# countertype/brotli-lib

Measured on AMD Instinct MI355X. Metric: encode+decode MB/s at q11 lgwin=22, higher is better.
Workload: dtype u8; 1 GPU; C4 per-GPU shard: 1024 x 1048576 B enwik-style text, q11 lgwin22 GENERIC, encode -> decode round trip (statuses and sizes checked); streams_per_gpu=1024, quality=11, lgwin=22, mode=0, parallelism=shard1

## Files before the change

brotli-lib_amd/csrc/enc_common.h:

```cpp
#pragma once
#include <hip/hip_runtime.h>
#include <stdint.h>

#include "common.h"
#include "parts.h"

#ifndef RFC_CONST
#define RFC_CONST static __device__ const
#endif
#include "rfc_tables.h"

namespace mib {
namespace enc {

constexpr uint32_t kSegBits = 16;
constexpr uint32_t kSeg = 1u << kSegBits;
#ifndef MIB_MAX_MATCHES
#define MIB_MAX_MATCHES 4
#endif
constexpr int kMaxMatches = MIB_MAX_MATCHES;
static_assert(kMaxMatches == 4 || kMaxMatches == 6 || kMaxMatches == 8, "records of 4, 6 or 8 entries");
constexpr int kMatchRec = kMaxMatches;
constexpr uint32_t kMatchLenSat = 255;
constexpr int kLongCopy = 200;
// ... 336 lines not shown
}
__device__ __forceinline__ uint32_t switch_bits(const Codes &cd, int cat, const Unit &u) {
  const int bc = block_count_code(u.sw_count[cat]);
  return cd.btd[cat][u.sw_code[cat]] + cd.bcd[cat][bc] + kBlkBits[bc];
}
__device__ __forceinline__ bool switch_at(const Unit &u, int cat, uint32_t q) { return u.sw_count[cat] && q == u.first[cat]; }
__device__ __forceinline__ bool lit_switch_at(const Unit &u, uint32_t lp) { return u.sw_count[0] && lp == u.first[0]; }

__device__ __forceinline__ uint32_t item_count(const Cmd &c) { return c.ins + 2; }

__device__ __forceinline__ uint32_t header_bits(const Codes &cd, const Cmd &c, const Unit &u, uint32_t q) {
  const int ic = ins_code(c.ins);
  const int cc = copy_code(c.copy ? c.copy : 2);
  uint32_t bits = cd.cd[u.type[1]][c.cmd_prefix] + kInsExtra[ic] + kCopyExtra[cc];
  if (switch_at(u, 1, q)) bits += switch_bits(cd, 1, u);
  return bits;
}
__device__ __forceinline__ int literal_tree(const uint16_t *cmap, const uint8_t *lut, const Unit &u, uint32_t p12) {
  return cmap[u.type[0] * kLitCtx + (lut[p12 & 0xFF] | lut[256 + (p12 >> 8)])];
}
__device__ __forceinline__ uint32_t dist_bits(const Codes &cd, const Mb &mb, const Cmd &c, const Unit &u, uint32_t q) {
  if (!c.copy || c.cmd_prefix < 128) return 0;
  uint32_t bits = cd.dd[mb.dist_cmap[u.type[2] * kDistCtx + dist_ctx(c.copy)]][c.dist_prefix & 0x3FF] + (c.dist_prefix >> 10);
  if (switch_at(u, 2, q)) bits += switch_bits(cd, 2, u);
  return bits;
}
__device__ __forceinline__ uint32_t item_bits(const Codes &cd, const Mb &mb, const uint16_t *cmap, const uint8_t *lut, const Job &jb,
                                              const Cmd &c, uint32_t p, const Seg &sg, const Unit *su, uint32_t q,
                                              uint32_t k) {
  if (k == 0) return header_bits(cd, c, su[unit_of(sg, p)], q);
  if (k > c.ins) return dist_bits(cd, mb, c, su[unit_of(sg, p)], q);
  const uint32_t lp = p + k - 1;
  const Unit &ul = su[unit_of(sg, lp)];
  return (lit_switch_at(ul, lp) ? switch_bits(cd, 0, ul) : 0u) + cd.ld[literal_tree(cmap, lut, ul, prev2(jb, lp))][jb.data[lp]];
}

template <int B>
struct ItemMap {
  uint32_t off[B + 1];
  __device__ __forceinline__ uint32_t find(uint32_t i, uint32_t nb) const {
    uint32_t lo = 0, hi = nb;
    while (hi - lo > 1) {
      const uint32_t mid = (lo + hi) >> 1;
      if (off[mid] <= i) lo = mid;
      else hi = mid;
    }
    return lo;
  }
};

void launch_dict_matches(hipStream_t st, const Job *jobs, int njobs, uint32_t span, const uint32_t *dict_tab,
                         const uint8_t *dict_data, uint32_t *matches);
void launch_cdict_matches(hipStream_t st, const Job *jobs, const uint32_t *pos_job, uint32_t total, uint32_t *matches);
void launch_find_matches(hipStream_t st, const Job *jobs, const uint32_t *pos_job, const SegRef *seg_ref,
                         const uint32_t *skeys, const uint32_t *svals, uint32_t total, int depth, uint32_t max_dist,
                         bool hist, bool parts, uint32_t *matches);
void launch_near_matches(hipStream_t st, const Job *jobs, const uint32_t *pos_job, const SegRef *seg_ref, uint32_t total,
                         uint32_t max_dist, bool hist, bool parts, uint32_t *matches);
void launch_lit_histo(hipStream_t st, const Job *jobs, const Seg *segs, int nsegs, uint32_t *lit_h);
void launch_hist_update(hipStream_t st, const Job *jobs, const uint32_t *pos_job, const uint32_t *skeys,
                        const uint32_t *svals, uint32_t total);
size_t cost_model_hist_bytes(int njobs);
void launch_cost_model(hipStream_t st, const Job *jobs, int njobs, const Seg *segs, int nsegs, const RawCmd *raw,
                       uint32_t *hist, CostModel *model);
void launch_dp(hipStream_t st, const Job *jobs, const Seg *segs, int nsegs, const uint32_t *lit_h, const CostModel *model,
               const uint32_t *matches, uint64_t *choice, bool cdict, bool font, const uint32_t *words, uint32_t *ring_hist,
               const Mb *mbs, int piece_shift);
void dp_launch_counts(unsigned long long out[4]);
size_t dp_ring_hist_bytes(int nsegs);
void launch_any_binary(hipStream_t st, const Job *jobs, int njobs, uint32_t *flag);
void launch_words(hipStream_t st, const Job *jobs, const uint32_t *pos_job, const SegRef *seg_ref, uint32_t total, uint32_t *words);
void launch_backtrack(hipStream_t st, const Job *jobs, Seg *segs, int nsegs, const uint64_t *choice, RawCmd *raw);
void launch_carry(hipStream_t st, Job *jobs, int njobs, Seg *segs, const Mb *mbs);
void launch_derive_segs(hipStream_t st, const Seg *segs, int nsegs, uint32_t sample, Seg *d_sample, Seg *pieces);
void launch_merge_pieces(hipStream_t st, const Job *jobs, Seg *segs, int nsegs, const Seg *pieces, RawCmd *raw);
void launch_rep(hipStream_t st, const Job *jobs, Seg *segs, int nsegs, const CostModel *model, RawCmd *raw, uint32_t *cnts);
size_t sort_ws_bytes(uint32_t total);
void launch_sort(hipStream_t st, const Job *jobs, const uint32_t *pos_job, int njobs, uint32_t total, int hb, void *ws,
                 uint32_t *tmp_k, uint32_t *tmp_v, uint32_t *skeys, uint32_t *svals);
void launch_codes(hipStream_t st, const Job *jobs, const Seg *segs, const Mb *mbs, int nsegs, const RawCmd *raw, Cmd *cmds,
                  uint32_t *cmd_pos, Unit *units, uint32_t *unit_h);
void launch_split(hipStream_t st, hipStream_t side, const Job *jobs, Mb *mbs, int nmbs, Unit *units,
                  const uint32_t *unit_h, Codes *codes, int max_units, int max_short_units);
void launch_histo(hipStream_t st, const Job *jobs, const Seg *segs, const Mb *mbs, int nsegs, const Cmd *cmds,
                  const uint32_t *cmd_pos, const Unit *units, uint32_t *hl, uint32_t *hc, uint32_t *hd);
void launch_dist_ring(hipStream_t st, Job *jobs, int njobs, const Seg *segs, const Cmd *cmds);
void launch_context_mode(hipStream_t st, const Job *jobs, Mb *mbs, int nmbs);
void launch_cluster(hipStream_t st, const Job *jobs, Mb *mbs, int nmbs, uint32_t *hl, uint32_t *hd);
void launch_huffman(hipStream_t st, hipStream_t side, const Job *jobs, Mb *mbs, int nmbs, const uint32_t *hl,
                    const uint32_t *hc, const uint32_t *hd, Codes *codes, uint8_t *trees, uint8_t *hdr);
void launch_sizes(hipStream_t st, const Job *jobs, Seg *segs, const Mb *mbs, int nsegs, const Cmd *cmds,
                  const uint32_t *cmd_pos, const Codes *codes, const Unit *units, uint32_t *tile_bits);
void launch_offsets(hipStream_t st, Job *jobs, int njobs, Mb *mbs, Seg *segs, uint8_t *out);
void launch_emit(hipStream_t st, const Job *jobs, const Mb *mbs, int nmbs, const Seg *segs, int nsegs, const Cmd *cmds,
                 const uint32_t *cmd_pos, const Codes *codes, const Unit *units, const uint32_t *tile_bits,
                 const uint8_t *trees, const uint8_t *hdr, uint8_t *out);
void launch_stored(hipStream_t st, Job *jobs, int njobs, uint8_t *out);
struct PushSum;
void launch_ring_scan(hipStream_t st, Job *jobs, int njobs, Seg *segs, int nsegs, const RawCmd *raw, PushSum *push);
void launch_part_index(hipStream_t st, const Job *jobs, int njobs, const Mb *mbs, const Seg *segs, int nsegs,
                       const Cmd *cmds, const Unit *units, PushSum *push, uint8_t *out);
size_t part_push_bytes();
void launch_pack(hipStream_t st, const Job *jobs, int njobs, uint64_t out_pos, uint64_t out_cap, uint64_t *dst_off,
                 const uint8_t *src, uint8_t *dst);

}
}
```

brotli-lib_amd/csrc/enc_entropy.hip:

```cpp
#include <hipcub/hipcub.hpp>
#include <cstdlib>
#include <algorithm>

#include "enc_common.h"

namespace mib {
namespace enc {

__global__ __launch_bounds__(64) void carry_kernel(Job *jobs, int njobs, Seg *segs, const Mb *mbs) {
  const int j = blockIdx.x, lane = threadIdx.x;
  if (j >= njobs) return;
  Job &jb = jobs[j];
  if (jb.uncompressed) return;
  uint32_t pd = (uint32_t)jb.dc_in[0];
  for (uint32_t m = 0; m < jb.nmb; m++) {
    const Mb &mb = mbs[jb.mb_base + m];
    uint32_t carry = 0;
    const uint32_t end = mb.first_seg + mb.nseg;
    for (uint32_t c0 = mb.first_seg; c0 < end; c0 += 64) {
      const uint32_t s = c0 + lane;
      const bool live = s < end;
      uint32_t ncmd = 0, tail = 0, last = 0;
      if (live) {
        ncmd = segs[s].ncmd;
// ... 138 lines not shown
    const uint32_t off = (uint32_t)(ex >> 35), total = (uint32_t)(tot >> 35);
    const uint32_t loff = (uint32_t)(ex >> 10) & 0x1FFFFFFu, nlits = (uint32_t)(tot >> 10) & 0x1FFFFFFu;
    const uint32_t rank = (uint32_t)ex & 0x3FFu, npush = (uint32_t)tot & 0x3FFu;
    const uint32_t pos = sh_run + off;
    if (push) sh_push[rank] = d;
    __syncthreads();
    uint32_t ring[4];
#pragma unroll
    for (int k = 0; k < 4; k++) ring[k] = (int)rank - 1 - k >= 0 ? sh_push[rank - 1 - k] : sh_ring[k - rank];
    uint32_t ring_after = 0;
    if (t < 4) ring_after = (int)npush - 1 - t >= 0 ? sh_push[npush - 1 - t] : sh_ring[t - npush];
    __syncthreads();
    if (t < 4) sh_ring[t] = ring_after;
    if (t == 0) sh_run += total;
    if (q < n) {
      Cmd c;
      c.ins = ins;
      c.copy = len;
      c.dist = d;
      c.dist_extra = 0;
      c.dist_prefix = 0;
      const int ic = ins_code(ins);
      const uint32_t u = unit_of(sg, pos);
      uint32_t *hu = sh_h + u * kSubHist;
      if (len) {
        const uint32_t dcode = is_word(jb, d) ? (d & ~kDictFlag) + 15 : d == prevd ? 0 : short_code(d, ring);
        uint32_t extra;
        const uint32_t dp = dist_prefix(dcode, (int)jb.ndirect, (int)jb.npostfix, &extra);
        c.dist_extra = extra;
        c.dist_prefix = (uint16_t)dp;
        c.cmd_prefix = (uint16_t)combine_codes(ic, copy_code(len), dcode == 0);
        if (c.cmd_prefix >= 128) {
          atomicAdd(&hu[256 + 704 + (dp & 0x3FF)], 1u);
          atomicAdd(&sh_n[u][2], 1u);
          atomicMin(&sh_first[u][2], q);
        }
      } else {
        c.cmd_prefix = (uint16_t)combine_codes(ic, 0, ic < 8);
      }
      atomicAdd(&hu[256 + c.cmd_prefix], 1u);
      atomicAdd(&sh_n[u][1], 1u);
      atomicMin(&sh_first[u][1], q);
      if (ins) {
        const uint32_t ulo = unit_of(sg, pos), uhi = unit_of(sg, pos + ins - 1);
        for (uint32_t v = ulo; v <= uhi; v++) {
          const uint32_t s0 = v == ulo ? pos : sg.start + (v << kSubBits);
          const uint32_t s1 = v == uhi ? pos + ins : sg.start + ((v + 1) << kSubBits);
          atomicAdd(&sh_n[v][0], s1 - s0);
          atomicMin(&sh_first[v][0], s0);
        }
      }
      out[q] = c;
      outp[q] = pos;
    }
    sh_pos[t] = pos;
    const uint32_t nb = min((uint32_t)NT, n - base);
    map.off[t] = loff;
    if (t == 0) map.off[nb] = nlits;
    __syncthreads();
    for (uint32_t i = t; i < nlits; i += NT) {
      const uint32_t j = map.find(i, nb);
      const uint32_t lp = sh_pos[j] + i - map.off[j];
      atomicAdd(&sh_h[unit_of(sg, lp) * kSubHist + jb.data[lp]], 1u);
    }
    __syncthreads();
  }
  const uint32_t u0 = blockIdx.x * kSubPerSeg;
  uint32_t *gh = unit_h + (size_t)u0 * kSubHist;
  for (int i = t; i < kSubPerSeg * kSubHist; i += NT) gh[i] = sh_h[i];
  if (t < kSubPerSeg) {
    Unit un;
    for (int c = 0; c < 3; c++) {
      un.nsym[c] = sh_n[t][c];
      un.first[c] = sh_first[t][c];
      un.sw_count[c] = 0;
      un.type[c] = 0;
      un.sw_code[c] = 0;
    }
    un.pad = 0;
    units[u0 + t] = un;
  }
}

template <int NT>
__global__ __launch_bounds__(NT) void histo_kernel(const Job *jobs, const Seg *segs, const Mb *mbs, const Cmd *cmds,
                                                       const uint32_t *cmd_pos, const Unit *units, uint32_t *hl,
                                                       uint32_t *hc, uint32_t *hd) {
  typedef hipcub::BlockScan<uint32_t, NT> Scan;
  __shared__ typename Scan::TempStorage scan_tmp;
  __shared__ uint32_t sh_l[kLitCtx * 256];
  __shared__ uint8_t ut[kSubPerSeg][3];
  __shared__ ItemMap<NT> map;
  __shared__ uint32_t sh_pos[NT], sh_ins[NT];
  uint32_t *sh_c = sh_l, *sh_d = sh_l + kMaxBT * 704;
  const Seg &sg = segs[blockIdx.x];
  const Job &jb = jobs[sg.job];
  if (jb.uncompressed) return;
  const Mb &mb = mbs[sg.mb];
  const int t = threadIdx.x;
  __shared__ uint8_t lut[512];
  for (int i = t; i < 512; i += NT) lut[i] = kRfcContextLut[(mb.ctx_mode << 9) + i];
  const Unit *un = units + (size_t)blockIdx.x * kSubPerSeg;
  if (t < kSubPerSeg * 3) ut[t / 3][t % 3] = un[t / 3].type[t % 3];
  for (int i = t; i < (int)mb.nbt[1] * 704; i += NT) sh_c[i] = 0;
  for (int i = t; i < (int)mb.nbt[2] * kDistCtx * 128; i += NT) sh_d[i] = 0;
  __syncthreads();
  const Cmd *c = cmds + sg.cmd_off;
  const uint32_t *cp = cmd_pos + sg.cmd_off;
  const uint32_t n = sg.ncmd + (sg.extra_ins ? 1 : 0);
  for (uint32_t q = t; q < n; q += NT) {
    const Cmd k = c[q];
    const uint32_t u = unit_of(sg, cp[q]);
    atomicAdd(&sh_c[ut[u][1] * 704 + k.cmd_prefix], 1u);
    if (k.copy && k.cmd_prefix >= 128) atomicAdd(&sh_d[(ut[u][2] * kDistCtx + dist_ctx(k.copy)) * 128 + (k.dist_prefix & 0x3FF)], 1u);
  }
  const uint32_t m = sg.mb;
  __syncthreads();
  for (int i = t; i < (int)mb.nbt[1] * 704; i += NT)
    if (sh_c[i]) atomicAdd(&hc[(size_t)m * kMaxBT * 704 + i], sh_c[i]);
  for (int i = t; i < (int)mb.nbt[2] * kDistCtx * 128; i += NT)
    if (sh_d[i]) atomicAdd(&hd[(size_t)m * kMaxBT * kDistCtx * 128 + i], sh_d[i]);
  __syncthreads();
  uint32_t present = 0;
  for (int u = 0; u < kSubPerSeg; u++) present |= 1u << ut[u][0];
  for (int ty = 0; ty < kMaxBT; ty++) {
    if (!(present >> ty & 1)) continue;
    for (int i = t; i < kLitCtx * 256; i += NT) sh_l[i] = 0;
    __syncthreads();
    for (uint32_t base = 0; base < n; base += NT) {
      const uint32_t q = base + t, nb = min((uint32_t)NT, n - base);
      uint32_t cnt = 0;
      if (q < n && c[q].ins) {
        const uint32_t pos = cp[q], ins = c[q].ins;
        sh_pos[t] = pos;
        sh_ins[t] = ins;
        const uint32_t ulo = unit_of(sg, pos), uhi = unit_of(sg, pos + ins - 1);
        for (uint32_t v = ulo; v <= uhi; v++)
          if (ut[v][0] == ty) {
            const uint32_t s0 = v == ulo ? pos : sg.start + (v << kSubBits);
            const uint32_t s1 = v == uhi ? pos + ins : sg.start + ((v + 1) << kSubBits);
            cnt += s1 - s0;
          }
      }
      uint32_t off, nlits;
      Scan(scan_tmp).ExclusiveSum(cnt, off, nlits);
      map.off[t] = off;
      if (t == 0) map.off[nb] = nlits;
      __syncthreads();
      for (uint32_t i = t; i < nlits; i += NT) {
        const uint32_t j = map.find(i, nb);
        const uint32_t pos = sh_pos[j], ins = sh_ins[j];
        const uint32_t ulo = unit_of(sg, pos), uhi = unit_of(sg, pos + ins - 1);
        uint32_t k = i - map.off[j], lp = pos;
        for (uint32_t v = ulo; v <= uhi; v++) {
          if (ut[v][0] != ty) continue;
          const uint32_t s0 = v == ulo ? pos : sg.start + (v << kSubBits);
          const uint32_t s1 = v == uhi ? pos + ins : sg.start + ((v + 1) << kSubBits);
          if (k < s1 - s0) {
            lp = s0 + k;
            break;
          }
          k -= s1 - s0;
        }
        const uint32_t p12 = prev2(jb, lp);
        atomicAdd(&sh_l[(lut[p12 & 0xFF] | lut[256 + (p12 >> 8)]) * 256 + jb.data[lp]], 1u);
      }
      __syncthreads();
    }
    uint32_t *dst = hl + ((size_t)m * kLitSlots + ty * kLitCtx) * 256;
    for (int i = t; i < kLitCtx * 256; i += NT)
      if (sh_l[i]) atomicAdd(&dst[i], sh_l[i]);
    __syncthreads();
  }
}

__device__ __forceinline__ float hist_cost(float bits, int nnz) {
  if (nnz <= 1) return 12.f;
  if (nnz <= 4) return bits + 20.f + 4.f * nnz;
  return bits + 40.f + 3.5f * nnz;
}

constexpr int kCluT = 1024;
constexpr int kCluPairs = kLitCtx * (kLitCtx - 1) / 2;
__device__ __forceinline__ int tri(int a, int b) { return a * (2 * kLitCtx - a - 1) / 2 + b - a - 1; }
#ifdef MIB_PROF
__device__ unsigned long long g_clu_prof[8];
#endif
__global__ __launch_bounds__(kCluT) void cluster_kernel(const Job *jobs, Mb *mbs, int nmbs, uint32_t *hl, uint32_t *hd,
                                                         int lit_cap, int kl, int kd) {
  constexpr int kMaxH = kLitCtx;
  __shared__ uint32_t h[kMaxH][257];
  __shared__ float cost[kMaxH];
  __shared__ float save[kCluPairs];
  __shared__ uint16_t pair_of[kCluPairs];
  __shared__ int alive[kMaxH], label[kMaxH];
  __shared__ float red_v[kCluT / 64];
  __shared__ int red_i[kCluT / 64];
  __shared__ int sh_best, sh_alive;
  __shared__ int rep_id[kMaxH];
  const int nb = kl + 4, m = blockIdx.x / nb, r0 = blockIdx.x % nb;
  Mb &mb = mbs[m];
  const Job &jb = jobs[mb.job];
  if (jb.uncompressed) return;
  const int t = threadIdx.x;
#ifdef MIB_PROF
  uint64_t cp[6] = {0, 0, 0, 0, 0, 0}, cp0 = __builtin_amdgcn_s_memtime();
#define CLMARK(k)                                         \
  do {                                                    \
    if (t == 0) {                                         \
      const uint64_t t_ = __builtin_amdgcn_s_memtime();   \
      cp[k] += t_ - cp0;                                  \
// ... 1925 lines not shown
    if (lane == 0) mb.bit_off = pos;
    uint64_t hb = lane < kTreeSlots ? mb.tree_bits[lane] : 0;
    for (int q = lane + 64; q < kTreeSlots; q += 64) hb += mb.tree_bits[q];
    for (int o = 32; o; o >>= 1) hb += __shfl_xor(hb, o);
    pos += mb.hdr_bits + hb;
    const uint32_t end = mb.first_seg + mb.nseg;
    for (uint32_t c0 = mb.first_seg; c0 < end; c0 += 64) {
      const uint32_t s = c0 + lane;
      const uint64_t bits = s < end ? segs[s].bits : 0;
      uint64_t inc = bits;
#pragma unroll
      for (int o = 1; o < 64; o <<= 1) {
        const uint64_t y = __shfl_up(inc, o);
        if (lane >= o) inc += y;
      }
      if (s < end) segs[s].bit_off = pos + inc - bits;
      pos += __shfl(inc, 63);
    }
    if (mb.is_last) pos = (pos + 7) & ~7ull;
  }
  if (lane != 0) return;
  const uint64_t trailer = pos;
  if (!jb.final_) pos = (pos + 6 + 7) & ~7ull;
  const uint64_t stored_bits = 8ull * ((uint64_t)jb.n + 5ull * ((jb.n >> 24) + 1) + 4);
  if (pos > stored_bits || (pos >> 3) + 8 > jb.out_cap) {
    jb.uncompressed = 2;
    for (int q = 0; q < 4; q++) jb.dc_out[q] = jb.dc_in[q];
    return;
  }
  if (!jb.final_) {
    uint32_t *w = reinterpret_cast<uint32_t *>(out + jb.out_off);
    const uint64_t v = 6ull << (trailer & 31);
    atomicOr(w + (trailer >> 5), (uint32_t)v);
    if ((uint32_t)(v >> 32)) atomicOr(w + (trailer >> 5) + 1, (uint32_t)(v >> 32));
  }
  jb.total_bits = pos;
}

void launch_carry(hipStream_t st, Job *jobs, int njobs, Seg *segs, const Mb *mbs) {
  hipLaunchKernelGGL(carry_kernel, dim3(njobs), dim3(64), 0, st, jobs, njobs, segs, mbs);
}
void launch_codes(hipStream_t st, const Job *jobs, const Seg *segs, const Mb *mbs, int nsegs, const RawCmd *raw, Cmd *cmds,
                  uint32_t *cmd_pos, Unit *units, uint32_t *unit_h) {
  static const int nt = knob("MIB_CODES_NT") ? atoi(knob("MIB_CODES_NT")) : 512;
  if (nt >= 512)
    hipLaunchKernelGGL(codes_kernel<512>, dim3(nsegs), dim3(512), 0, st, jobs, segs, mbs, raw, cmds, cmd_pos, units, unit_h);
  else
    hipLaunchKernelGGL(codes_kernel<256>, dim3(nsegs), dim3(256), 0, st, jobs, segs, mbs, raw, cmds, cmd_pos, units, unit_h);
}
void launch_split(hipStream_t st, hipStream_t side, const Job *jobs, Mb *mbs, int nmbs, Unit *units,
                  const uint32_t *unit_h, Codes *codes, int max_units, int max_short_units) {
  const SplitK sk = split_k();
  const bool wide_short = std::max(sk.k[0], std::max(sk.k[1], sk.k[2])) > 4;
  const bool wide_long = std::max(std::min(sk.k[0], 4), std::max(sk.k[1], sk.k[2])) > 4;
  const bool narrow = std::min(sk.k[0], std::min(sk.k[1], sk.k[2])) <= 4 || max_units > kSplitWideUnits || sk.k[0] > 4;
  const size_t lds4 = (size_t)std::max(1, std::min(max_units, kMaxUnits)) * 4 * sizeof(float);
  const size_t lds8 = (size_t)std::max(1, std::min(wide_long ? max_units : max_short_units, kMaxUnits)) * kMaxBT * sizeof(float);
  static const bool attr = [] {
    hipFuncSetAttribute((const void *)split_kernel<1024, 4>, hipFuncAttributeMaxDynamicSharedMemorySize, kMaxUnits * 4 * 4);
    hipFuncSetAttribute((const void *)split_kernel<256, 4>, hipFuncAttributeMaxDynamicSharedMemorySize, kMaxUnits * 4 * 4);
    hipFuncSetAttribute((const void *)split_kernel<1024, kMaxBT>, hipFuncAttributeMaxDynamicSharedMemorySize, kMaxUnits * kMaxBT * 4);
    hipFuncSetAttribute((const void *)split_kernel<256, kMaxBT>, hipFuncAttributeMaxDynamicSharedMemorySize, kMaxUnits * kMaxBT * 4);
    return true;
  }();
  (void)attr;
  const bool few = nmbs * 3 <= 256;
  if (narrow) {
    if (few) hipLaunchKernelGGL((split_kernel<1024, 4>), dim3(nmbs * 3), dim3(1024), lds4, side, jobs, mbs, nmbs, units, unit_h, codes, sk);
    else hipLaunchKernelGGL((split_kernel<256, 4>), dim3(nmbs * 3), dim3(256), lds4, side, jobs, mbs, nmbs, units, unit_h, codes, sk);
  }
  if (wide_short || wide_long) {
    if (few) hipLaunchKernelGGL((split_kernel<1024, kMaxBT>), dim3(nmbs * 3), dim3(1024), lds8, st, jobs, mbs, nmbs, units, unit_h, codes, sk);
    else hipLaunchKernelGGL((split_kernel<256, kMaxBT>), dim3(nmbs * 3), dim3(256), lds8, st, jobs, mbs, nmbs, units, unit_h, codes, sk);
  }
  static const bool widen = !knob("MIB_SPLIT_WIDEN") || atoi(knob("MIB_SPLIT_WIDEN")) != 0;
  if (widen && narrow && std::max(sk.k[1], sk.k[2]) <= 4) {
    SplitK wk = sk;
    wk.widen = 1;
    const size_t ldsw = (size_t)std::max(1, std::min(max_units, kMaxUnits)) * kMaxBT * sizeof(float);
    if (few) hipLaunchKernelGGL((split_kernel<1024, kMaxBT>), dim3(nmbs * 3), dim3(1024), ldsw, side, jobs, mbs, nmbs, units, unit_h, codes, wk);
    else hipLaunchKernelGGL((split_kernel<256, kMaxBT>), dim3(nmbs * 3), dim3(256), ldsw, side, jobs, mbs, nmbs, units, unit_h, codes, wk);
  }
}
void launch_histo(hipStream_t st, const Job *jobs, const Seg *segs, const Mb *mbs, int nsegs, const Cmd *cmds,
                  const uint32_t *cmd_pos, const Unit *units, uint32_t *hl, uint32_t *hc, uint32_t *hd) {
  static const int nt = knob("MIB_HISTO_NT") ? atoi(knob("MIB_HISTO_NT")) : 1024;
  if (nt >= 1024)
    hipLaunchKernelGGL(histo_kernel<1024>, dim3(nsegs), dim3(1024), 0, st, jobs, segs, mbs, cmds, cmd_pos, units, hl, hc, hd);
  else if (nt >= 512)
    hipLaunchKernelGGL(histo_kernel<512>, dim3(nsegs), dim3(512), 0, st, jobs, segs, mbs, cmds, cmd_pos, units, hl, hc, hd);
  else
    hipLaunchKernelGGL(histo_kernel<256>, dim3(nsegs), dim3(256), 0, st, jobs, segs, mbs, cmds, cmd_pos, units, hl, hc, hd);
}
void launch_dist_ring(hipStream_t st, Job *jobs, int njobs, const Seg *segs, const Cmd *cmds) {
  hipLaunchKernelGGL(dist_ring_kernel, dim3((njobs + 63) / 64), dim3(64), 0, st, jobs, njobs, segs, cmds);
}
void launch_context_mode(hipStream_t st, const Job *jobs, Mb *mbs, int nmbs) {
  static const int force = knob("MIB_CTX_MODE") ? atoi(knob("MIB_CTX_MODE")) & 3 : -1;
  hipLaunchKernelGGL(context_mode_kernel, dim3(nmbs), dim3(64), 0, st, jobs, mbs, nmbs, force);
}
constexpr int kLitTreeCap = 24;
int lit_tree_cap() {
  static const int cap = knob("MIB_LIT_TREES") ? std::min(kMaxLitTrees, std::max(1, atoi(knob("MIB_LIT_TREES")))) : kLitTreeCap;
  return cap;
}
void launch_cluster(hipStream_t st, const Job *jobs, Mb *mbs, int nmbs, uint32_t *hl, uint32_t *hd) {
  const SplitK sk = split_k();
  static const int kd = knob("MIB_TYPE_SIZING") ? sk.k[2] : kMaxBT;
  hipLaunchKernelGGL(cluster_kernel, dim3(nmbs * (sk.k[0] + 4)), dim3(kCluT), 0, st, jobs, mbs, nmbs, hl, hd, lit_tree_cap(),
                     sk.k[0], kd);
}
void launch_huffman(hipStream_t st, hipStream_t side, const Job *jobs, Mb *mbs, int nmbs, const uint32_t *hl,
                    const uint32_t *hc, const uint32_t *hd, Codes *codes, uint8_t *trees, uint8_t *hdr) {
  const SplitK sk = split_k();
  static const int kc = knob("MIB_TYPE_SIZING") ? sk.k[1] : kMaxBT, kdt = knob("MIB_TYPE_SIZING") ? sk.k[2] : kMaxBT;
  (void)kdt;
  const int nl = std::max(lit_tree_cap(), sk.k[0]), nr = nl + 4 + 4 * kDistCtx;
  hipLaunchKernelGGL(huffman_kernel<704>, dim3(nmbs * nr), dim3(64), 0, st, jobs, mbs, nmbs, hl, hc, hd, codes, trees, nl, kc, nr);
  hipLaunchKernelGGL(mb_header_kernel, dim3(nmbs), dim3(64), 0, side, jobs, mbs, nmbs, hdr, codes);
}
void launch_sizes(hipStream_t st, const Job *jobs, Seg *segs, const Mb *mbs, int nsegs, const Cmd *cmds,
                  const uint32_t *cmd_pos, const Codes *codes, const Unit *units, uint32_t *tile_bits) {
  static const int nt = knob("MIB_SIZES_NT") ? atoi(knob("MIB_SIZES_NT")) : 512;
  static const int target = knob("MIB_EMIT_BLOCKS") ? std::max(1, atoi(knob("MIB_EMIT_BLOCKS"))) : 2048;
  const dim3 grid(nsegs, std::min(kEmitTiles, std::max(1, (target + nsegs - 1) / std::max(nsegs, 1))));
  if (nt >= 512)
    hipLaunchKernelGGL(sizes_kernel<512>, grid, dim3(512), 0, st, jobs, segs, mbs, cmds, cmd_pos, codes, units, tile_bits);
  else
    hipLaunchKernelGGL(sizes_kernel<256>, grid, dim3(256), 0, st, jobs, segs, mbs, cmds, cmd_pos, codes, units, tile_bits);
}
void launch_offsets(hipStream_t st, Job *jobs, int njobs, Mb *mbs, Seg *segs, uint8_t *out) {
  hipLaunchKernelGGL(offsets_kernel, dim3(njobs), dim3(64), 0, st, jobs, njobs, mbs, segs, out);
}

}
}
#ifdef MIB_PROF
extern "C" int mib_debug_read_huff_prof(unsigned long long *out) {
  hipMemcpyFromSymbol(out, HIP_SYMBOL(mib::enc::g_huff_prof), sizeof(unsigned long long) * 12);
  unsigned long long z[12] = {0, 0, 0, 0, 0, 0, 0, 0, 0, 0, 0, 0};
  hipMemcpyToSymbol(HIP_SYMBOL(mib::enc::g_huff_prof), z, sizeof(z));
  return 0;
}
#endif
#ifdef MIB_PROF
extern "C" int mib_debug_read_split_prof(unsigned long long *out) {
  hipMemcpyFromSymbol(out, HIP_SYMBOL(mib::enc::g_split_prof), sizeof(unsigned long long) * 8);
  unsigned long long z[8] = {0, 0, 0, 0, 0, 0, 0, 0};
  hipMemcpyToSymbol(HIP_SYMBOL(mib::enc::g_split_prof), z, sizeof(z));
  return 0;
}
#endif
#ifdef MIB_PROF
extern "C" int mib_debug_read_clu_prof(unsigned long long *out) {
  hipMemcpyFromSymbol(out, HIP_SYMBOL(mib::enc::g_clu_prof), sizeof(unsigned long long) * 8);
  unsigned long long z[8] = {0, 0, 0, 0, 0, 0, 0, 0};
  hipMemcpyToSymbol(HIP_SYMBOL(mib::enc::g_clu_prof), z, sizeof(z));
  return 0;
}
#endif
```

brotli-lib_amd/csrc/encode.hip:

```cpp
#include <hip/hip_runtime.h>
#include <stdio.h>
#include <stdlib.h>
#include <string.h>

#include <algorithm>
#include <atomic>
#include <memory>
#include <mutex>
#include <thread>
#include <vector>

#include "enc_common.h"

extern "C" void mib_ctx_add_time(mib_ctx *c, const char *name, double ms);
extern "C" int mib_ctx_profiling(mib_ctx *c);
extern "C" void **mib_ctx_enc_ws(mib_ctx *c);
extern "C" void **mib_ctx_lane_ws(mib_ctx *c, int l);
extern "C" void *mib_ctx_lane_stream(mib_ctx *c, int l);
extern "C" uint8_t *mib_ctx_stage(mib_ctx *c, int slot, uint64_t need);

using namespace mib;
using namespace mib::enc;

extern "C" mib_ctx *mib_default_ctx(void);
// ... 713 lines not shown
  d.cdict_len = 0;
  d.cdict_tail4 = 0;
  if (!one_shot) {
    d.hdr_lgwin = (uint32_t)prm.lgwin;
  } else if (n == 0) {
    d.hdr_lgwin = 10;
  } else if (prm.quality == 0 || n < 64) {
    int lg = 10;
    if (n > 1) {
      int c = 0;
      while ((1ull << c) < n) c++;
      lg = std::max(10, std::min(24, c + 1));
    }
    d.hdr_lgwin = (uint32_t)lg;
  } else {
    d.hdr_lgwin = (uint32_t)prm.lgwin;
  }
}

struct DevDict {
  uint8_t *d = nullptr;
  uint32_t n = 0, tail4 = 0;
  int upload(const uint8_t *h, uint64_t len, hipStream_t st) {
    if (!h || len < 4) return 0;
    if (len >= (1ull << 31)) return MIB_E_INVALID_ARG;
    if (hipMalloc(&d, len + 64) != hipSuccess) return MIB_E_OUT_OF_MEMORY;
    CK(hipMemcpyAsync(d, h, len, hipMemcpyHostToDevice, st));
    n = (uint32_t)len;
    tail4 = (uint32_t)h[len - 4] | ((uint32_t)h[len - 3] << 8) | ((uint32_t)h[len - 2] << 16) | ((uint32_t)h[len - 1] << 24);
    return 0;
  }
  void attach(StreamDesc &sd) const {
    sd.cdict = d;
    sd.cdict_len = n;
    sd.cdict_tail4 = tail4;
  }
  void release() {
    if (d) hipFree(d);
    d = nullptr;
    n = 0;
  }
};

constexpr uint64_t kMaxChunk = 256ull << 20;
constexpr uint64_t kStage = 8ull << 20;
constexpr uint64_t kStageBudget = 256ull << 20;
std::atomic<uint64_t> g_stage_bytes{0};
std::atomic<int> g_live_encoders{0};
uint64_t out_bound(uint64_t n) { return n + n / 8 + 4096 + 16 + sizeof(PartHead) + ((n + kSeg - 1) / kSeg) * sizeof(PartEntry); }

}

struct mib_encoder {
  mib_enc_opts opts;
  uint64_t pend = 0;
  bool started = false;
  bool finished = false;
  int32_t dc[4] = {4, 11, 15, 16};
  uint32_t prev_bytes = 0;
  uint64_t window = 1 << 22;
  uint64_t block = 1 << 16;
  uint64_t chunk = 0;
  bool chunk_fixed = true;
  int device = -1;
  uint8_t *buf[2] = {nullptr, nullptr};
  uint64_t buf_cap = 0;
  int cur = 0;
  uint64_t hist = 0;
  uint64_t abs = 0;
  uint64_t obytes = 0;
  uint32_t *tab = nullptr;
  std::vector<uint8_t> dict;
  DevDict ddict;
  uint8_t *stage = nullptr;
  uint64_t staged = 0;
};
extern "C" {

void mib_force_no_dp_cache(int off) { __atomic_store_n(&g_no_dp_cache, off ? 1 : 0, __ATOMIC_RELAXED); }
void mib_debug_dp_launches(uint64_t out[4]) {
  unsigned long long v[4];
  enc::dp_launch_counts(v);
  for (int q = 0; q < 4; q++) out[q] = v[q];
}

void mib_encode_ws_free(void *p) {
  Workspace *ws = reinterpret_cast<Workspace *>(p);
  if (!ws) return;
  if (ws->buf) hipFree(ws->buf);
  if (ws->side) hipStreamDestroy(ws->side);
  if (ws->fork_ev) hipEventDestroy(ws->fork_ev);
  if (ws->join_ev) hipEventDestroy(ws->join_ev);
  delete ws;
}
int mib_live_encoders(void) { return g_live_encoders.load(); }
void mib_encode_ws_trim(void **p, uint64_t keep) {
  Workspace *ws = reinterpret_cast<Workspace *>(*p);
  if (!ws) return;
  ws->quiet = ws->need > keep ? 0 : ws->quiet + 1;
  ws->need = 0;
  if (ws->cap > keep && ws->quiet >= 4) {
    mib_encode_ws_free(ws);
    *p = nullptr;
  }
}

int mib_ctx_encode(mib_ctx *c, const mib_enc_opts *o, const uint8_t *d_in, const uint64_t *in_offsets, size_t k,
                   uint8_t *d_out, uint64_t out_cap, uint64_t *out_offsets, void *stream) {
  if (!c || !out_offsets || (k && (!d_in || !in_offsets || !d_out))) return MIB_E_INVALID_ARG;
  if (mib_ctx_ready(c) != 0) return MIB_E_NO_DEVICE;
  hipStream_t st = stream ? (hipStream_t)stream : (hipStream_t)mib_ctx_stream_of(c);
  mib_ctx_clear_times(c);
  Params prm = make_params(o);
  DevDict dd;
  int rc = o ? dd.upload(o->dict, o->dict_len, st) : 0;
  if (rc) return rc;
  std::vector<StreamDesc> sd(k);
  for (size_t i = 0; i < k; i++) {
    if (in_offsets[i + 1] < in_offsets[i] || in_offsets[i + 1] - in_offsets[i] >= (1ull << 31)) {
      dd.release();
      return MIB_E_INVALID_ARG;
    }
    fill_desc(sd[i], d_in + in_offsets[i], in_offsets[i + 1] - in_offsets[i], prm, true);
    dd.attach(sd[i]);
  }
  rc = encode_streams(c, o, sd.data(), k, d_out, out_cap, out_offsets, nullptr, st);
  hipStreamSynchronize(st);
  dd.release();
  return rc;
}

struct DefaultLock {
  DefaultLock() { mib_default_lock(1); }
  ~DefaultLock() { mib_default_lock(0); }
};

static int encode_host(const mib_span *in, size_t k, const mib_enc_opts *o, mib_buf *out, int *status) {
  DefaultLock use;
  mib_ctx *c = mib_default_ctx();
  if (!c) return MIB_E_NO_DEVICE;
  CK(hipSetDevice(mib_ctx_device_of(c)));
  hipStream_t st = (hipStream_t)mib_ctx_stream_of(c);
  Params prm = make_params(o);
  std::vector<uint64_t> ioff(k + 1, 0);
  uint64_t cap = 0;
  for (size_t i = 0; i < k; i++) {
    ioff[i + 1] = ioff[i] + ((in[i].size + 255) & ~(uint64_t)255);
    cap += out_bound(in[i].size);
  }
  uint8_t *d_in = mib_ctx_stage(c, 0, ioff[k] + 64), *d_out = mib_ctx_stage(c, 1, cap + 64);
  if (!d_in || !d_out) return MIB_E_OUT_OF_MEMORY;
  hipMemsetAsync(d_in, 0, ioff[k] + 64, st);
  std::vector<HostPiece> up;
  for (size_t i = 0; i < k; i++)
    if (in[i].size) up.push_back(HostPiece{d_in + ioff[i], in[i].data, in[i].size});
  int rc = ctx_upload(c, st, up.data(), up.size());
  if (rc) return rc;
  DevDict dd;
  rc = o ? dd.upload(o->dict, o->dict_len, st) : 0;
  if (rc) return rc;
  std::vector<StreamDesc> sd(k);
  for (size_t i = 0; i < k; i++) {
    fill_desc(sd[i], d_in + ioff[i], in[i].size, prm, true);
    dd.attach(sd[i]);
  }
  std::vector<uint64_t> ooff(k + 1, 0);
// ... 382 lines not shown
```

brotli-lib_amd/python/brotli_amd/__init__.py:

```python
import ctypes
import os

__all__ = ['brotliEncode', 'BrotliEncoder', 'brotliDecode', 'BrotliDecoder', 'brotliDecodedSize', 'EncoderMode', 'BrotliError',
           'encode_batch', 'decode_batch', 'encoder_update_batch', 'decoder_update_batch', 'decoder_finish_batch',
           'decoder_update_batch_device', 'decoder_finish_batch_device', 'MORE_OUTPUT', 'DeviceContext', 'library_path',
           'woff2_decode']

_PKG = os.path.dirname(os.path.dirname(os.path.dirname(os.path.abspath(__file__))))
_LIB_PATH = os.environ.get('BROTLI_AMD_LIB') or os.path.join(_PKG, 'libbrotli_amd.so')


def library_path():
    return _LIB_PATH


class EncoderMode:
    GENERIC = 0
    TEXT = 1
    FONT = 2


class BrotliError(Exception):
    def __init__(self, message, code=None):
        super().__init__(message)
# ... 377 lines not shown
        raise ValueError('decoder_update_batch: %d decoders, %d chunks' % (k, len(chunks)))
    keep = [_in(b) for b in chunks]
    hs = (ctypes.c_void_p * k)(*[d._h for d in decoders])
    spans = (_Span * k)(*[_Span(_addr(a) if n else None, n) for a, n, _ in keep])
    outs = (_Buf * k)()
    st = (ctypes.c_int * k)()
    return _decoder_batch_results(decoders, _L().mib_decoder_update_batch(hs, spans, k, outs, st), outs, st)


def decoder_finish_batch(decoders):
    k = len(decoders)
    hs = (ctypes.c_void_p * k)(*[d._h for d in decoders])
    outs = (_Buf * k)()
    st = (ctypes.c_int * k)()
    return _decoder_batch_results(decoders, _L().mib_decoder_finish_batch(hs, k, outs, st), outs, st)


MORE_OUTPUT = 1


def _device_offsets(what, offsets, k):
    if len(offsets) != k + 1:
        raise ValueError('%s: %d decoders need %d offsets, got %d' % (what, k, k + 1, len(offsets)))
    return (ctypes.c_uint64 * (k + 1))(*offsets)


def decoder_update_batch_device(decoders, d_in, in_offsets, d_out, out_offsets):
    k = len(decoders)
    ioff = _device_offsets('decoder_update_batch_device', in_offsets, k)
    ooff = _device_offsets('decoder_update_batch_device', out_offsets, k)
    hs = (ctypes.c_void_p * k)(*[d._h for d in decoders])
    sizes = (ctypes.c_uint64 * k)()
    st = (ctypes.c_int * k)()
    rc = _L().mib_decoder_update_batch_device(hs, d_in, ioff, k, d_out, ooff, sizes, st)
    if rc:
        raise _err(rc)
    return list(sizes), list(st)


def decoder_finish_batch_device(decoders, d_out, out_offsets):
    k = len(decoders)
    ooff = _device_offsets('decoder_finish_batch_device', out_offsets, k)
    hs = (ctypes.c_void_p * k)(*[d._h for d in decoders])
    sizes = (ctypes.c_uint64 * k)()
    st = (ctypes.c_int * k)()
    rc = _L().mib_decoder_finish_batch_device(hs, k, d_out, ooff, sizes, st)
    if rc:
        raise _err(rc)
    return list(sizes), list(st)


def debug_copy_batch(srcs, dsts, sizes):
    k = len(sizes)
    rc = _L().mib_debug_copy_batch((ctypes.c_void_p * k)(*srcs), (ctypes.c_void_p * k)(*dsts), (ctypes.c_uint64 * k)(*sizes), k)
    if rc:
        raise _err(rc)


def encode_batch(buffers, options=None, gpus=None):
    k = len(buffers)
    keep = [_in(b) for b in buffers]
    spans = (_Span * k)(*[_Span(_addr(a), n) for a, n, _ in keep])
    outs = (_Buf * k)()
    st = (ctypes.c_int * k)()
    if gpus is None:
        rc = _L().mib_encode_batch(spans, k, ctypes.byref(_opts(options)), outs, st)
    else:
        rc = _L().mib_encode_batch_n(spans, k, ctypes.byref(_opts(options)), int(gpus), outs, st)
    if rc:
        raise _err(rc)
    res = [_take(outs[i]) for i in range(k)]
    for i in range(k):
        if st[i]:
            raise _err(st[i])
    return res


def debug_dp_launches():
    out = (ctypes.c_uint64 * 4)()
    _L().mib_debug_dp_launches(out)
    return {1: out[0], 2: out[1], 4: out[2], 8: out[3]}


def debug_match_records(buffers, options=None):
    import numpy as np
    k = len(buffers)
    keep = [_in(b) for b in buffers]
    spans = (_Span * k)(*[_Span(_addr(a), n) for a, n, _ in keep])
    outs = (_Buf * k)()
    rc = _L().mib_debug_match_records(spans, k, ctypes.byref(_opts(options)), outs)
    if rc:
        raise _err(rc)
    res = []
    for i in range(k):
        n = keep[i][1]
        a = np.frombuffer(_take(outs[i]), dtype='<u4')
        res.append(a.reshape(n, -1) if n else a.reshape(0, 4))
    return res


def decode_batch(buffers, gpus=None):
    k = len(buffers)
    keep = [_in(b) for b in buffers]
    spans = (_Span * k)(*[_Span(_addr(a), n) for a, n, _ in keep])
    outs = (_Buf * k)()
    st = (ctypes.c_int * k)()
    if gpus is None:
        rc = _L().mib_decode_batch(spans, k, outs, st)
    else:
        rc = _L().mib_decode_batch_n(spans, k, int(gpus), outs, st)
    if rc:
        raise _err(rc)
    return [(_take(outs[i]) if st[i] == 0 else _err(st[i])) for i in range(k)]


def woff2_transform_glyf(ttf):
    data = _bytes(ttf)
    buf = _Buf()
    rc = _L().mib_woff2_transform_glyf(data, len(data), ctypes.byref(buf))
    if rc:
        raise _err(rc)
    return _take(buf)


def woff2_transform_hmtx(ttf):
    data = _bytes(ttf)
    buf = _Buf()
    rc = _L().mib_woff2_transform_hmtx(data, len(data), ctypes.byref(buf))
    if rc:
        raise _err(rc)
    if not buf.size:
        _L().mib_buf_free(ctypes.byref(buf))
        return None
    return _take(buf)


def woff2_reconstruct_glyf(data):
    data = _bytes(data)
    glyf, loca = _Buf(), _Buf()
    rc = _L().mib_woff2_reconstruct_glyf(data, len(data), ctypes.byref(glyf), ctypes.byref(loca))
    if rc:
        raise _err(rc)
    return _take(glyf), _take(loca)


def woff2_reconstruct_hmtx(data, glyf, loca, num_glyphs, num_hmetrics):
    data, glyf, loca = _bytes(data), _bytes(glyf), _bytes(loca)
    if not 0 <= int(num_glyphs) <= 0xFFFFFFFF or not 0 <= int(num_hmetrics) <= 0xFFFFFFFF:
        raise _err(-101)
    buf = _Buf()
    rc = _L().mib_woff2_reconstruct_hmtx(data, len(data), glyf, len(glyf), loca, len(loca), int(num_glyphs),
                                         int(num_hmetrics), ctypes.byref(buf))
    if rc:
        raise _err(rc)
    return _take(buf)


def woff2_decode(data):
    data = _bytes(data)
    buf = _Buf()
    rc = _L().mib_woff2_decode(data, len(data), ctypes.byref(buf))
    if rc:
        raise _err(rc)
    return _take(buf)


# ... 89 lines not shown
```

include/brotli_amd.h:

```cpp
#ifndef BROTLI_AMD_H_
#define BROTLI_AMD_H_
#include <stddef.h>
#include <stdint.h>
#ifdef __cplusplus
extern "C" {
#endif

#define MIB_MODE_GENERIC 0
#define MIB_MODE_TEXT 1
#define MIB_MODE_FONT 2

#define MIB_E_NO_DEVICE (-100)
#define MIB_E_INVALID_ARG (-101)
#define MIB_E_OUT_OF_MEMORY (-102)
#define MIB_E_OUTPUT_LIMIT (-103)
#define MIB_E_NEED_SPACE (-104)
#define MIB_E_JS_RANGE_ERROR (-105)
#define MIB_E_JS_TYPE_ERROR (-106)
#define MIB_E_NO_PROGRESS (-107)

typedef struct {
  int quality;
  int lgwin;
  int mode;
  uint64_t size_hint;
  const uint8_t *dict;
  uint64_t dict_len;
  uint64_t stream_chunk;
} mib_enc_opts;

typedef struct { uint8_t *data; size_t size; } mib_buf;
typedef struct { const uint8_t *data; size_t size; } mib_span;

void mib_enc_opts_default(mib_enc_opts *o);

int mib_init(int device);
const char *mib_strerror(int code);

int mib_encode(const uint8_t *in, size_t n, const mib_enc_opts *o, mib_buf *out);

int mib_decode(const uint8_t *in, size_t n, const uint8_t *dict, size_t dict_n, int64_t max_out,
               int64_t exact_out, mib_buf *out);

int64_t mib_decoded_size(const uint8_t *in, size_t n);

typedef struct mib_encoder mib_encoder;
mib_encoder *mib_encoder_new(const mib_enc_opts *o);
int mib_encoder_update(mib_encoder *e, const uint8_t *in, size_t n, mib_buf *out);
int mib_encoder_finish(mib_encoder *e, mib_buf *out);
void mib_encoder_free(mib_encoder *e);
int mib_encoder_update_batch(mib_encoder *const *e, const mib_span *in, size_t k, mib_buf *out);

typedef struct {
  const uint8_t *dict;
  uint64_t dict_len;
  int64_t max_out;
  uint64_t out_window;
} mib_dec_opts;
void mib_dec_opts_default(mib_dec_opts *o);
typedef struct mib_decoder mib_decoder;
mib_decoder *mib_decoder_new(const mib_dec_opts *o);
int mib_decoder_update(mib_decoder *d, const uint8_t *in, size_t n, mib_buf *out);
int mib_decoder_finish(mib_decoder *d, mib_buf *out);
int mib_decoder_is_finished(const mib_decoder *d);
void mib_decoder_free(mib_decoder *d);
void mib_decoder_stats(const mib_decoder *d, uint64_t *passes, uint64_t *redecoded);
void mib_force_decoder_build(int four_per_cu);
int mib_decoder_update_batch(mib_decoder *const *d, const mib_span *in, size_t k, mib_buf *out, int *status);
int mib_decoder_finish_batch(mib_decoder *const *d, size_t k, mib_buf *out, int *status);
#define MIB_DEC_MORE_OUTPUT 1
int mib_decoder_update_batch_device(mib_decoder *const *d, const uint8_t *d_in, const uint64_t *in_offsets, size_t k,
                                    uint8_t *d_out, const uint64_t *out_offsets, uint64_t *out_sizes, int *status);
int mib_decoder_finish_batch_device(mib_decoder *const *d, size_t k, uint8_t *d_out, const uint64_t *out_offsets,
                                    uint64_t *out_sizes, int *status);
uint64_t mib_decoder_held_output(const mib_decoder *d);
int mib_debug_copy_batch(const uint8_t *const *d_src, uint8_t *const *d_dst, const uint64_t *n, size_t k);
void mib_decoder_batch_stats(uint64_t *launches);
void mib_decoder_batch_times(double *ms, int n);
void mib_force_decoder_grid(int max_blocks);

int mib_encode_batch(const mib_span *in, size_t k, const mib_enc_opts *o, mib_buf *out, int *status);
int mib_decode_batch(const mib_span *in, size_t k, mib_buf *out, int *status);
int mib_encode_batch_n(const mib_span *in, size_t k, const mib_enc_opts *o, int n_gpus, mib_buf *out, int *status);
int mib_decode_batch_n(const mib_span *in, size_t k, int n_gpus, mib_buf *out, int *status);
int mib_device_count(void);
int64_t mib_selftest_lds_atomic_order(int trials);
void mib_force_ballot_rank(int force);
void mib_force_shards(int force);
void mib_force_no_dp_cache(int off);
void mib_debug_dp_launches(uint64_t out[4]);
int mib_debug_match_records(const mib_span *in, size_t k, const mib_enc_opts *o, mib_buf *out);

void mib_buf_free(mib_buf *b);
typedef void *(*mib_alloc_func)(void *opaque, size_t size);
typedef void (*mib_free_func)(void *opaque, void *address);
void mib_set_allocator(mib_alloc_func alloc_func, mib_free_func free_func, void *opaque);

typedef struct mib_ctx mib_ctx;
mib_ctx *mib_ctx_new(int device);
void mib_ctx_free(mib_ctx *c);
int mib_ctx_encode(mib_ctx *c, const mib_enc_opts *o, const uint8_t *d_in, const uint64_t *in_offsets,
                   size_t k, uint8_t *d_out, uint64_t out_cap, uint64_t *out_offsets, void *stream);
int mib_ctx_decode(mib_ctx *c, const uint8_t *d_in, const uint64_t *in_offsets, size_t k, uint8_t *d_out,
                   const uint64_t *out_offsets, int64_t *out_sizes, int *status, void *stream);
typedef struct { char name[32]; double ms; uint32_t launches; } mib_kernel_time;
int mib_ctx_kernel_times(mib_ctx *c, mib_kernel_time *out, int max);
void mib_ctx_set_profiling(mib_ctx *c, int on);
mib_ctx *mib_default_ctx(void);
void mib_ctx_clear_times(mib_ctx *c);
int mib_woff2_transform_glyf(const uint8_t *ttf, size_t n, mib_buf *out);
int mib_woff2_transform_hmtx(const uint8_t *ttf, size_t n, mib_buf *out);
int mib_woff2_reconstruct_glyf(const uint8_t *tglyf, size_t n, mib_buf *glyf, mib_buf *loca);
int mib_woff2_reconstruct_hmtx(const uint8_t *thmtx, size_t n, const uint8_t *glyf, size_t glyf_n,
                               const uint8_t *loca, size_t loca_n, uint32_t num_glyphs,
                               uint32_t num_hmetrics, mib_buf *out);
int mib_woff2_decode(const uint8_t *woff2, size_t n, mib_buf *sfnt);
int mib_debug_sfnt_assemble(uint32_t flavor, const uint32_t *tags, const mib_span *tables,
                            const uint8_t *d_src_misalign, size_t k, mib_buf *sfnt);

void mib_part_stats(mib_ctx *c, uint64_t *parallel, uint64_t *fallback);

#ifdef __cplusplus
}
#endif
#endif
```

Before: 3516 MB/s.

## Count literal histograms by position bitmap instead of per-command scan

Adds a by-position literal histogram path, now the default. Each command marks the boundaries of its insert range in a shared-memory XOR bitmap, and a block-wide prefix-XOR turns those marks into a per-byte literal mask. Literals are then counted by walking set bits per bitmap word, with separate handling for insert ranges that spill outside the segment. This replaces the old BlockScan/ItemMap command walk and is meant to cut scan and synchronisation overhead and improve load balance. In exchange it adds a 64 KB/32-word bitmap to LDS, which may reduce occupancy, and it relies on a subtle boundary-handling scheme. The old path stays available behind a knob.

Result: no change. 3535 MB/s (median of 6 runs) (+0.6%).

```diff
diff --git a/brotli-lib_amd/csrc/enc_common.h b/brotli-lib_amd/csrc/enc_common.h
--- a/brotli-lib_amd/csrc/enc_common.h
+++ b/brotli-lib_amd/csrc/enc_common.h
@@ -442,6 +442,8 @@
                   uint32_t *cmd_pos, Unit *units, uint32_t *unit_h);
 void launch_split(hipStream_t st, hipStream_t side, const Job *jobs, Mb *mbs, int nmbs, Unit *units,
                   const uint32_t *unit_h, Codes *codes, int max_units, int max_short_units);
+void force_histo_walk(int by_command);
+void histo_launch_counts(unsigned long long out[2]);
 void launch_histo(hipStream_t st, const Job *jobs, const Seg *segs, const Mb *mbs, int nsegs, const Cmd *cmds,
                   const uint32_t *cmd_pos, const Unit *units, uint32_t *hl, uint32_t *hc, uint32_t *hd);
 void launch_dist_ring(hipStream_t st, Job *jobs, int njobs, const Seg *segs, const Cmd *cmds);
diff --git a/brotli-lib_amd/csrc/enc_entropy.hip b/brotli-lib_amd/csrc/enc_entropy.hip
--- a/brotli-lib_amd/csrc/enc_entropy.hip
+++ b/brotli-lib_amd/csrc/enc_entropy.hip
@@ -244,16 +244,21 @@
   }
 }
 
-template <int NT>
+constexpr uint32_t kBmWords = kSeg / 32;
+template <int NT, bool BYPOS>
 __global__ __launch_bounds__(NT) void histo_kernel(const Job *jobs, const Seg *segs, const Mb *mbs, const Cmd *cmds,
                                                        const uint32_t *cmd_pos, const Unit *units, uint32_t *hl,
                                                        uint32_t *hc, uint32_t *hd) {
   typedef hipcub::BlockScan<uint32_t, NT> Scan;
-  __shared__ typename Scan::TempStorage scan_tmp;
+  constexpr int NW = BYPOS ? 1 : NT;
+  __shared__ typename std::conditional<BYPOS, uint32_t, typename Scan::TempStorage>::type scan_tmp;
   __shared__ uint32_t sh_l[kLitCtx * 256];
   __shared__ uint8_t ut[kSubPerSeg][3];
-  __shared__ ItemMap<NT> map;
-  __shared__ uint32_t sh_pos[NT], sh_ins[NT];
+  __shared__ ItemMap<NW> map;
+  __shared__ uint32_t sh_pos[NW], sh_ins[NW];
+  __shared__ uint32_t bm[BYPOS ? kBmWords : 1];
+  __shared__ uint32_t sh_out[4];
+  __shared__ uint32_t sh_par[NT / 64];
   uint32_t *sh_c = sh_l, *sh_d = sh_l + kMaxBT * 704;
   const Seg &sg = segs[blockIdx.x];
   const Job &jb = jobs[sg.job];
@@ -266,15 +271,37 @@
   if (t < kSubPerSeg * 3) ut[t / 3][t % 3] = un[t / 3].type[t % 3];
   for (int i = t; i < (int)mb.nbt[1] * 704; i += NT) sh_c[i] = 0;
   for (int i = t; i < (int)mb.nbt[2] * kDistCtx * 128; i += NT) sh_d[i] = 0;
+  if (BYPOS) {
+    for (uint32_t i = t; i < kBmWords; i += NT) bm[i] = 0;
+    if (t < 4) sh_out[t] = 0;
+  }
   __syncthreads();
   const Cmd *c = cmds + sg.cmd_off;
   const uint32_t *cp = cmd_pos + sg.cmd_off;
   const uint32_t n = sg.ncmd + (sg.extra_ins ? 1 : 0);
+  const uint32_t seg_len = min(sg.end - sg.start, kSeg);
   for (uint32_t q = t; q < n; q += NT) {
     const Cmd k = c[q];
-    const uint32_t u = unit_of(sg, cp[q]);
+    const uint32_t pos = cp[q];
+    const uint32_t u = unit_of(sg, pos);
     atomicAdd(&sh_c[ut[u][1] * 704 + k.cmd_prefix], 1u);
     if (k.copy && k.cmd_prefix >= 128) atomicAdd(&sh_d[(ut[u][2] * kDistCtx + dist_ctx(k.copy)) * 128 + (k.dist_prefix & 0x3FF)], 1u);
+    if (BYPOS && k.ins) {
+      const uint32_t pe = pos + k.ins, s0 = sg.start, s1 = sg.start + seg_len;
+      if (pos < s0) {
+        sh_out[0] = pos;
+        sh_out[1] = min(pe, s0);
+      }
+      if (pe > s1) {
+        sh_out[2] = max(pos, s1);
+        sh_out[3] = pe;
+      }
+      const uint32_t lo = max(pos, s0), hi = min(pe, s1);
+      if (lo < hi) {
+        atomicXor(&bm[(lo - s0) >> 5], 1u << ((lo - s0) & 31));
+        if (hi < s0 + kSeg) atomicXor(&bm[(hi - s0) >> 5], 1u << ((hi - s0) & 31));
+      }
+    }
   }
   const uint32_t m = sg.mb;
   __syncthreads();
@@ -285,10 +312,49 @@
   __syncthreads();
   uint32_t present = 0;
   for (int u = 0; u < kSubPerSeg; u++) present |= 1u << ut[u][0];
+  if constexpr (BYPOS) {
+    constexpr uint32_t K = kBmWords / NT;
+    static_assert(K >= 1 && K * NT == kBmWords, "bitmap words per thread");
+    uint32_t w[K], carry = 0;
+#pragma unroll
+    for (uint32_t j = 0; j < K; j++) {
+      uint32_t x = bm[t * K + j];
+      x ^= x << 1;
+      x ^= x << 2;
+      x ^= x << 4;
+      x ^= x << 8;
+      x ^= x << 16;
+      w[j] = carry ? ~x : x;
+      carry = w[j] >> 31;
+    }
+    const uint64_t odd = __ballot(carry != 0);
+    const uint32_t lane = t & 63, wave = t >> 6;
+    if (lane == 0) sh_par[wave] = (uint32_t)__popcll(odd) & 1u;
+    __syncthreads();
+    uint32_t before = (uint32_t)__popcll(odd & ((1ull << lane) - 1ull)) & 1u;
+    for (uint32_t v = 0; v < wave; v++) before ^= sh_par[v];
+#pragma unroll
+    for (uint32_t j = 0; j < K; j++) bm[t * K + j] = before ? ~w[j] : w[j];
+  }
   for (int ty = 0; ty < kMaxBT; ty++) {
     if (!(present >> ty & 1)) continue;
     for (int i = t; i < kLitCtx * 256; i += NT) sh_l[i] = 0;
     __syncthreads();
+    if constexpr (BYPOS) {
+      auto count = [&](uint32_t lp) {
+        const uint32_t p12 = prev2(jb, lp);
+        atomicAdd(&sh_l[(lut[p12 & 0xFF] | lut[256 + (p12 >> 8)]) * 256 + jb.data[lp]], 1u);
+      };
+      for (uint32_t i = t; i < kBmWords; i += NT) {
+        if (ut[i >> (kSubBits - 5)][0] != ty) continue;
+        for (uint32_t x = bm[i]; x; x &= x - 1) count(sg.start + i * 32 + (uint32_t)__ffs((int)x) - 1);
+      }
+      if (ut[0][0] == ty)
+        for (uint32_t lp = sh_out[0] + t; lp < sh_out[1]; lp += NT) count(lp);
+      if (sh_out[2] < sh_out[3] && ut[unit_of(sg, sh_out[2])][0] == ty)
+        for (uint32_t lp = sh_out[2] + t; lp < sh_out[3]; lp += NT) count(lp);
+      __syncthreads();
+    } else
     for (uint32_t base = 0; base < n; base += NT) {
       const uint32_t q = base + t, nb = min((uint32_t)NT, n - base);
       uint32_t cnt = 0;
@@ -2380,15 +2446,25 @@
     else hipLaunchKernelGGL((split_kernel<256, kMaxBT>), dim3(nmbs * 3), dim3(256), ldsw, side, jobs, mbs, nmbs, units, unit_h, codes, wk);
   }
 }
+static int g_histo_walk = knob("MIB_HISTO_WALK") ? atoi(knob("MIB_HISTO_WALK")) : 0;
+static unsigned long long g_histo_launches[2];
 void launch_histo(hipStream_t st, const Job *jobs, const Seg *segs, const Mb *mbs, int nsegs, const Cmd *cmds,
                   const uint32_t *cmd_pos, const Unit *units, uint32_t *hl, uint32_t *hc, uint32_t *hd) {
   static const int nt = knob("MIB_HISTO_NT") ? atoi(knob("MIB_HISTO_NT")) : 1024;
-  if (nt >= 1024)
-    hipLaunchKernelGGL(histo_kernel<1024>, dim3(nsegs), dim3(1024), 0, st, jobs, segs, mbs, cmds, cmd_pos, units, hl, hc, hd);
+  const bool walk = __atomic_load_n(&g_histo_walk, __ATOMIC_RELAXED) != 0;
+  __atomic_fetch_add(&g_histo_launches[walk ? 1 : 0], 1ull, __ATOMIC_RELAXED);
+  if (walk)
+    hipLaunchKernelGGL((histo_kernel<1024, false>), dim3(nsegs), dim3(1024), 0, st, jobs, segs, mbs, cmds, cmd_pos, units, hl, hc, hd);
+  else if (nt >= 1024)
+    hipLaunchKernelGGL((histo_kernel<1024, true>), dim3(nsegs), dim3(1024), 0, st, jobs, segs, mbs, cmds, cmd_pos, units, hl, hc, hd);
   else if (nt >= 512)
-    hipLaunchKernelGGL(histo_kernel<512>, dim3(nsegs), dim3(512), 0, st, jobs, segs, mbs, cmds, cmd_pos, units, hl, hc, hd);
+    hipLaunchKernelGGL((histo_kernel<512, true>), dim3(nsegs), dim3(512), 0, st, jobs, segs, mbs, cmds, cmd_pos, units, hl, hc, hd);
   else
-    hipLaunchKernelGGL(histo_kernel<256>, dim3(nsegs), dim3(256), 0, st, jobs, segs, mbs, cmds, cmd_pos, units, hl, hc, hd);
+    hipLaunchKernelGGL((histo_kernel<256, true>), dim3(nsegs), dim3(256), 0, st, jobs, segs, mbs, cmds, cmd_pos, units, hl, hc, hd);
+}
+void force_histo_walk(int by_command) { __atomic_store_n(&g_histo_walk, by_command ? 1 : 0, __ATOMIC_RELAXED); }
+void histo_launch_counts(unsigned long long out[2]) {
+  for (int q = 0; q < 2; q++) out[q] = __atomic_load_n(&g_histo_launches[q], __ATOMIC_RELAXED);
 }
 void launch_dist_ring(hipStream_t st, Job *jobs, int njobs, const Seg *segs, const Cmd *cmds) {
   hipLaunchKernelGGL(dist_ring_kernel, dim3((njobs + 63) / 64), dim3(64), 0, st, jobs, njobs, segs, cmds);
diff --git a/brotli-lib_amd/csrc/encode.hip b/brotli-lib_amd/csrc/encode.hip
--- a/brotli-lib_amd/csrc/encode.hip
+++ b/brotli-lib_amd/csrc/encode.hip
@@ -819,6 +819,12 @@
   unsigned long long v[4];
   enc::dp_launch_counts(v);
   for (int q = 0; q < 4; q++) out[q] = v[q];
+}
+void mib_force_histo_walk(int by_command) { enc::force_histo_walk(by_command); }
+void mib_debug_histo_launches(uint64_t out[2]) {
+  unsigned long long v[2];
+  enc::histo_launch_counts(v);
+  for (int q = 0; q < 2; q++) out[q] = v[q];
 }
 
 void mib_encode_ws_free(void *p) {
diff --git a/brotli-lib_amd/python/brotli_amd/__init__.py b/brotli-lib_amd/python/brotli_amd/__init__.py
--- a/brotli-lib_amd/python/brotli_amd/__init__.py
+++ b/brotli-lib_amd/python/brotli_amd/__init__.py
@@ -483,6 +483,16 @@
     return {1: out[0], 2: out[1], 4: out[2], 8: out[3]}
 
 
+def force_histo_walk(by_command):
+    _L().mib_force_histo_walk(1 if by_command else 0)
+
+
+def debug_histo_launches():
+    out = (ctypes.c_uint64 * 2)()
+    _L().mib_debug_histo_launches(out)
+    return {'position': out[0], 'command': out[1]}
+
+
 def debug_match_records(buffers, options=None):
     import numpy as np
     k = len(buffers)
diff --git a/include/brotli_amd.h b/include/brotli_amd.h
--- a/include/brotli_amd.h
+++ b/include/brotli_amd.h
@@ -89,6 +89,8 @@
 void mib_force_shards(int force);
 void mib_force_no_dp_cache(int off);
 void mib_debug_dp_launches(uint64_t out[4]);
+void mib_force_histo_walk(int by_command);
+void mib_debug_histo_launches(uint64_t out[2]);
 int mib_debug_match_records(const mib_span *in, size_t k, const mib_enc_opts *o, mib_buf *out);
 
 void mib_buf_free(mib_buf *b);
```
